# Orca0917/fine-grained-emotional-control-of-tts

Measured on AMD Instinct MI355X. Metric: train mel-frames/sec at B=32, 80-bin mel; 1/2/4/8 MI355X, higher is better.
Workload: dtype bf16; 1 GPU; FastSpeech2 train step (fwd+loss+bwd+allreduce+AdamW), B=32/GPU, T_phon_max=200, T_mel_max=977, D=384 F=1536 6+6 FFT layers, 80 mels; global_batch=32, seq_len=977, parallelism=dp1

## Files before the change

fine-grained-emotional-control-of-tts_amd/csrc/gemm.hip:

```cpp
#include <type_traits>

#include "fs2_cdna.h"
#include "fs2_launch.h"

#include <cstdlib>
#include <cstring>

namespace {

#ifdef FS2_EXPERIMENTS
#define XFLAGS(p) ((p).g4_flags)
#else
#define XFLAGS(p) 0
#endif

constexpr int BM = 128, BN = 128, NT = 256;
constexpr int TILE_BYTES = 128 * 128;

struct GemmP {
  int M, N, K, kvalid, mvalid, nvalid;
  const char* A; long lda; const char* B; long ldb;
  int conv_mode, conv_t, conv_kw, conv_c, conv_p;
  int conv_dil;
  char* C; long ldc; int c_fp32; int c_conv_kw;
// ... 2 lines not shown
  const float* row_scale;
  const char* residual; long ldr;
  const float* row_scale_post;
  int accumulate; int split_k; int k_per_split;
  long split_stride;
  int g4_flags;
  int batch_div;
  long sA1, sA2, sB1, sB2, sC1, sC2, sR1, sR2;
  int tiles_m, tiles_n;
  int vec_ok;
  int vec_align;
  int c_row_t, c_row_pad;
  int max_ctas;
  int a_bytes, b_bytes;
  int a_kw;
  const int32_t* k_eff;
};

__device__ __forceinline__ u32x4 add_bf16x8(u32x4 a, u32x4 b) {
  u32x4 r;
#pragma unroll
  for (int w = 0; w < 4; ++w) {
    float a0 = __builtin_bit_cast(float, a[w] << 16), a1 = __builtin_bit_cast(float, a[w] & 0xffff0000u);
    float b0 = __builtin_bit_cast(float, b[w] << 16), b1 = __builtin_bit_cast(float, b[w] & 0xffff0000u);
    bf16 r0 = (bf16)(a0 + b0), r1 = (bf16)(a1 + b1);
    r[w] = (unsigned)__builtin_bit_cast(unsigned short, r0) |
           ((unsigned)__builtin_bit_cast(unsigned short, r1) << 16);
  }
  return r;
}
__device__ __forceinline__ u32x4 add_f32x4(u32x4 a, u32x4 b) {
  const f32x4 fa = __builtin_bit_cast(f32x4, a), fb = __builtin_bit_cast(f32x4, b);
// ... 673 lines not shown
  const int z = p.split_k > 1 ? 0 : blockIdx.z;
  const long zb = z / p.batch_div, zh = z - zb * p.batch_div;
  const char* Ab = p.A + (zb * p.sA1 + zh * p.sA2) * 2;
  const char* Bb = p.B + (zb * p.sB1 + zh * p.sB2) * 2;
  const int K = p.K;
  const int kva = min(K, p.kvalid);
  const int amode = CM >= 0 ? CM : ((p.conv_mode == 1 || p.conv_mode == 4 || p.conv_mode == 5) ? p.conv_mode : 0);
  const int nk_all = (K + 63) / 64;
  int kt0 = 0, kt1 = nk_all;
  if (p.split_k > 1) {
    const int kps = (nk_all + p.split_k - 1) / p.split_k;
    kt0 = blockIdx.z * kps;
    kt1 = min(nk_all, kt0 + kps);
  }
  const bool bconv3 = B3 >= 0 ? B3 == 1 : p.conv_mode == 3;
  const bool tap_uniform = CM > 0 ? true : (CM == 0 ? false : amode && (p.conv_c % 64) == 0);
  const int rpu = amode == 4 ? p.conv_t + 2 * p.conv_p : p.conv_t;

  const i32x4 rsA = make_rsrc(Ab), rsB = make_rsrc(Bb);
  int avo[4];
  int abt[4], at[4], alc[4];
  bool aval[4];
#pragma unroll
  for (int i = 0; i < 4; ++i) {
    if constexpr (AK) {
      const int r = (wave * 4 + i) * 8 + (lane >> 3);
      alc[i] = (lane & 7) ^ (r & 7);
      const int row = m0 + r;
      aval[i] = row < p.M;
      const int rr = aval[i] ? row : 0;
// ... 126 lines not shown
        int ts = t + blc[i] - p.conv_p;
        ts = ts < 0 ? -ts : (ts >= p.conv_t ? 2 * (p.conv_t - 1) - ts : ts);
        const bool ok = bval[i] && k0 + bkr[i] < kva;
        const int vo = ok ? bvo[i] + (int)(((long)b * p.conv_t + ts) * p.ldb * 2) : BUF_OOB;
        blds16(rsB, vo, 0, lb + (wave * 2 + i) * 1024);
      }
    }
  };

  f32x4 acc[4][4];
#pragma unroll
  for (int i = 0; i < 4; ++i)
#pragma unroll
    for (int j = 0; j < 4; ++j) acc[i][j] = f32x4{0.f, 0.f, 0.f, 0.f};

  const int nk = kt1 - kt0;
  if (nk > 0) issue(kt0, 0);
  if (nk > 1) issue(kt0 + 1, 1);
  for (int it = 0; it < nk; ++it) {
    if (it + 1 < nk) asm volatile("s_waitcnt vmcnt(6)" ::: "memory");
    else asm volatile("s_waitcnt vmcnt(0)" ::: "memory");
    asm volatile("s_waitcnt lgkmcnt(0)" ::: "memory");
    __builtin_amdgcn_s_barrier();
    __builtin_amdgcn_sched_barrier(0);
    if (it + 2 < nk) issue(kt0 + it + 2, (it + 2) % 3);
    const char* la = smem + (it % 3) * BIG_STAGE;
    const char* lb = la + BIG_A;
    bf16x8 af[2][4], bfr[2][4];
#pragma unroll
    for (int s = 0; s < 2; ++s)
#pragma unroll
      for (int i = 0; i < 4; ++i) {
        af[s][i] = AK ? frag_bf16_kmajor(la, wm * 64 + i * 16, s, lane)
                      : frag_bf16_mnmajor_asm<512>(la, wm * 64 + i * 16, s, lane);
        bfr[s][i] = BKM ? frag_bf16_kmajor(lb, wn * 64 + i * 16, s, lane)
                        : frag_bf16_mnmajor_asm<256>(lb, wn * 64 + i * 16, s, lane);
      }
    if constexpr (!AK || !BKM) {
      asm volatile("s_waitcnt lgkmcnt(0)" ::: "memory");
#pragma unroll
// ... 67 lines not shown
  const int z = p.split_k > 1 ? 0 : blockIdx.z;
  const long zb = z / p.batch_div, zh = z - zb * p.batch_div;
  const char* Ab = p.A + (zb * p.sA1 + zh * p.sA2) * 2;
  const char* Bb = p.B + (zb * p.sB1 + zh * p.sB2) * 2;
  const int K = p.K;
  const int kva = min(K, p.kvalid);
  const int amode = CM >= 0 ? CM : ((p.conv_mode == 1 || p.conv_mode == 4 || p.conv_mode == 5) ? p.conv_mode : 0);
  const int nk_all = (K + 63) / 64;
  int kt0 = 0, kt1 = nk_all;
  if (p.split_k > 1) {
    const int kps = (nk_all + p.split_k - 1) / p.split_k;
    kt0 = blockIdx.z * kps;
    kt1 = min(nk_all, kt0 + kps);
  }
  const bool bconv3 = B3 >= 0 ? B3 == 1 : p.conv_mode == 3;
  const bool tap_uniform = CM > 0 ? true : (CM == 0 ? false : amode && (p.conv_c % 32) == 0);
  const int rpu = amode == 4 ? p.conv_t + 2 * p.conv_p : p.conv_t;

  const i32x4 rsA = make_rsrc(Ab), rsB = make_rsrc(Bb);
  int avo[2];
  int abt[2], at[2], ac[2];
  bool aval[2];
#pragma unroll
  for (int i = 0; i < 2; ++i) {
    const int piece = wave * 2 + i;
    if constexpr (AK) {
      const int r = piece * 16 + (lane >> 2);
      ac[i] = (lane & 3) ^ g4_fsw(r);
      const int row = m0 + r;
      aval[i] = row < p.M;
// ... 129 lines not shown
      const int dk = k0 - b_k;
      b_k = k0;
#pragma unroll
      for (int i = 0; i < 2; ++i) {
        int t = bt[i] + dk, b = bb[i];
        while (t >= p.conv_t) { t -= p.conv_t; ++b; }
        bt[i] = t; bb[i] = b;
        int ts = t + bc[i] - p.conv_p;
        ts = ts < 0 ? -ts : (ts >= p.conv_t ? 2 * (p.conv_t - 1) - ts : ts);
        const bool ok = bval[i] && k0 + bkr[i] < kva;
        const int vo = ok ? bvo[i] + (int)(((long)b * p.conv_t + ts) * p.ldb * 2) : BUF_OOB;
        blds16(rsB, vo, 0, dst + (wave * 2 + i) * 1024);
      }
    }
  };
  auto issue = [&](int it, int reg) {
    const int k0 = (kt0 + it) * 64 + (reg >> 1) * 32;
    char* dst = smem + (it & 1) * G4_SLOT + reg * G4_REG;
    if ((reg & 1) == 0) issueA(dst, k0);
    else issueB(dst, k0);
  };

  f32x4 acc[8][4];
#pragma unroll
  for (int i = 0; i < 8; ++i)
#pragma unroll
    for (int j = 0; j < 4; ++j) acc[i][j] = f32x4{0.f, 0.f, 0.f, 0.f};

  const int nk = kt1 - kt0;
  if (nk > 0) {
    issue(0, 1); issue(0, 0); issue(0, 3); issue(0, 2);
  }
  if (nk > 1) {
    issue(1, 1); issue(1, 0);
    asm volatile("s_waitcnt vmcnt(8)" ::: "memory");
  } else {
    asm volatile("s_waitcnt vmcnt(4)" ::: "memory");
  }
  __builtin_amdgcn_s_barrier();
  const bool stag = !(XFLAGS(p) & 1);
  const bool prio = !(XFLAGS(p) & 2);
  const bool nowait = XFLAGS(p) & 4;
  const bool noissue = XFLAGS(p) & 8;
  const int grp = stag ? wr : 1;
// ... 1518 lines not shown
  }
  constexpr int BIG_MIN_TILES = 60;
  const bool use_big = p.conv_mode != 2 &&
                       ((p.vec_ok && p.split_k <= 1 && tiles_big * batch >= BIG_MIN_TILES) ||
                        (slices && p.vec_ok && tiles_big * p.split_k >= 160) ||
                        (wgrad && tiles_big * split_big >= 160));
  if (!use_big) { pl.kernel = k128; return 0; }
  q.g4_flags = fs2_exp_int("FS2_BIG_FLAGS", 0);
  q.tiles_m = (p.M + BBM - 1) / BBM;
  if (wgrad) split_wgrad(split_big);
  pl.grid = dim3(q.tiles_m * q.tiles_n, 1, wgrad ? q.split_k : (slices ? p.split_k : gz));
  pl.kernel = K_BIG + tile_variant(ak, bk, conv_variant(q, 64), q.conv_mode);
  return 0;
}

int plan(const fs2_gemm_desc* d, GemmArgs& a, GemmPlan& pl) {
  const int rc = validate(d, a);
  return rc ? rc : plan_gemm(a, pl);
}

int launch(const GemmPlan& pl, hipStream_t s) {
  const GemmKernel& k = KERNELS[pl.kernel];
  hipLaunchKernelGGL(k.fn, pl.grid, dim3(k.block), 0, s, pl.p);
  FS2_CHECK_LAUNCH();
  return 0;
}

}

extern "C" int fs2_gemm(const fs2_gemm_desc* d, void* stream) {
  GemmArgs a;
  GemmPlan pl;
  if (const int rc = plan(d, a, pl)) return rc < 0 ? rc : 0;
  hipStream_t s = (hipStream_t)stream;
  const int oes = a.p.c_fp32 ? 4 : (a.dtype == FS2_BF16 ? 2 : 4);
  if (d->split_stride > 0)
    for (int z = a.p.split_k; z < d->split_k; ++z)
      if (hipMemset2DAsync(a.p.C + (long)z * d->split_stride * oes, a.p.ldc * oes, 0,
                           (size_t)a.p.nvalid * oes, a.p.mvalid, s) != hipSuccess)
        return FS2_EINVAL;
  return launch(pl, s);
}

extern "C" int fs2_gemm_plan(const fs2_gemm_desc* d, fs2_gemm_plan_info* out) {
  if (!out) return FS2_EINVAL;
  *out = fs2_gemm_plan_info{};
  GemmArgs a;
  GemmPlan pl;
  if (const int rc = plan(d, a, pl)) return rc < 0 ? rc : 0;
  std::strncpy(out->kernel, KERNELS[pl.kernel].name, sizeof(out->kernel) - 1);
  out->grid[0] = (int)pl.grid.x; out->grid[1] = (int)pl.grid.y; out->grid[2] = (int)pl.grid.z;
  out->block = KERNELS[pl.kernel].block;
  out->tiles_m = pl.p.tiles_m; out->tiles_n = pl.p.tiles_n;
  out->split_k = pl.p.split_k; out->k_per_split = pl.p.k_per_split;
  out->vec_ok = pl.p.vec_ok; out->accumulate = pl.p.accumulate;
  return 0;
}
```

fine-grained-emotional-control-of-tts_amd/csrc/norm.hip:

```cpp
#include <cstdlib>
#include <algorithm>
#include "fs2_launch.h"

namespace {

constexpr int MAXJ = 16;

template <bool DPP>
__device__ __forceinline__ float wsum(float v) {
  if constexpr (DPP) return wave_sum_dpp(v);
  else return wave_sum(v);
}

struct LnFwdP {
  const char* x; long ldx; const char* r; long ldr; float p_r; uint32_t salt_r;
  char* s_out; const float* gamma; const float* beta; float eps; int do_tanh;
  float p_o; uint32_t salt_o; const float* row_mask; const char* post_add; long ldp;
  char* y; long ldy; float* mean; float* rstd; int M, D; uint32_t seed;
  char* img; int img_t, img_p;
};

template <typename T>
__global__ void __launch_bounds__(256) ln_fwd_kernel(LnFwdP p) {
  const int lane = threadIdx.x & 63;
// ... 881 lines not shown
      const long v = (long)len[b] + halo;
      const int e = (int)(v < 0 ? 0 : (v > T ? T : v));
      w = fs2_km_width(b, e, T, P);
      if (end) end[b] = e;
    }
#pragma unroll
    for (int d = 1; d < 64; d <<= 1) {
      const int o = __shfl_up(w, d, 64);
      if (lane >= d) w += o;
    }
    if (offs && b < B) offs[b + 1] = carry + w;
    carry += __shfl(w, 63, 64);
  }
  if (offs)
    for (int i = B + 1 + lane; i < noffs; i += 64) offs[i] = 0x7fffffff;
}

__global__ void __launch_bounds__(256) pad_rows_kernel(const bf16* X, long ldx, int B, int T,
                                                       int C8, int P, int reflect, bf16* out,
                                                       long ldo, unsigned n8) {
  const unsigned idx = blockIdx.x * 256u + threadIdx.x;
  if (idx >= n8) return;
  const unsigned r = idx / (unsigned)C8;
  const int c = (int)(idx - r * (unsigned)C8) * 8;
  const unsigned L = (unsigned)(T + 2 * P);
  const unsigned b = r / L;
  const int i = (int)(r - b * L) - P;
  u32x4 v = {0u, 0u, 0u, 0u};
  if ((int)b < B) {
    const int t = reflect ? reflect_idx(i, T) : i;
// ... 233 lines not shown
                            ksplit, dtype, stream);
}

extern "C" int fs2_grad_tail_bounds(const int64_t* len, int B, int T, int halo, int P,
                                    int32_t* end, int32_t* offs, int noffs, void* stream) {
  if (B <= 0) return 0;
  if (!len || T <= 0 || halo < 0 || P < 0 || (!end && !offs)) return FS2_EINVAL;
  if (offs && (noffs < (B + 1 + 15) / 16 * 16 + 16 || (long)B * (T + 2L * P) >= 0x7fffffffL))
    return FS2_EINVAL;
  hipLaunchKernelGGL(grad_tail_bounds_kernel, dim3(1), dim3(64), 0, (hipStream_t)stream, len, B, T,
                     halo, P, end, offs, noffs);
  FS2_CHECK_LAUNCH();
  return 0;
}

extern "C" int fs2_pad_rows(const void* X, int64_t ldx, int B, int T, int C, int P, int reflect,
                            int tail, void* out, int64_t ldo, int dtype, void* stream) {
  if (B <= 0 || T <= 0 || C <= 0) return 0;
  if (dtype != FS2_BF16 || !X || !out || P < 0 || tail < 0 || (reflect && P >= T))
    return FS2_EINVAL;
  if ((C % 8) || (ldx % 8) || (ldo % 8) || ldo < C || ldx < C || !aligned16(X) || !aligned16(out))
    return FS2_EALIGN;
  const long rows = (long)B * (T + 2 * P) + tail;
  const long n8 = rows * (C / 8);
  if (n8 >= 0x7fffffffL || rows * ldo >= 0x7fffffffL) return FS2_EINVAL;
  hipLaunchKernelGGL(pad_rows_kernel, dim3((unsigned)((n8 + 255) / 256)), dim3(256), 0,
                     (hipStream_t)stream, (const bf16*)X, (long)ldx, B, T, C / 8, P, reflect,
                     (bf16*)out, (long)ldo, (unsigned)n8);
  FS2_CHECK_LAUNCH();
  return 0;
// ... 2 lines not shown
```

fine-grained-emotional-control-of-tts_amd/fastspeech2/_native.py:

```python

import ctypes
import os

import torch

_HERE = os.path.dirname(os.path.abspath(__file__))
LIB_PATH = os.environ.get("FS2_HIP_LIB", os.path.join(_HERE, "libfs2_hip.so"))
EXPERIMENTS = os.path.basename(LIB_PATH).startswith("libfs2_hip_exp")


def exp_flag(name, default=False):
    if not EXPERIMENTS:
        return default
    v = os.environ.get(name)
    return default if v is None else v not in ("", "0")


def exp_int(name, default):
    if not EXPERIMENTS:
        return default
    v = os.environ.get(name)
    return default if v is None else int(v)

F32 = 0
# ... 63 lines not shown
        ("O", ctypes.c_int), ("C", ctypes.c_int), ("KW", ctypes.c_int), ("w_okc", ctypes.c_int),
        ("ldf", ctypes.c_int), ("ldb", ctypes.c_int), ("tile0", ctypes.c_int),
        ("tiles_k", ctypes.c_int),
    ]


P = ctypes.c_void_p
I = ctypes.c_int
I64 = ctypes.c_int64
U32 = ctypes.c_uint32
Fl = ctypes.c_float

SIGNATURES = {
    "fs2_gemm": (I, [ctypes.POINTER(GemmDesc), P]),
    "fs2_gemm_plan": (I, [ctypes.POINTER(GemmDesc), ctypes.POINTER(GemmPlanInfo)]),
    "fs2_colsum": (I, [P, I64, I, I, I, P, I, P, P]),
    "fs2_conv_fold": (I, [P, I, I64, I, I, I, I, P, I64, P, I64, P, P, I, P]),
    "fs2_colsum_workspace_floats": (I64, [I, I]),
    "fs2_sum_slices": (I, [P, I, I64, I64, P, I, P]),
    "fs2_pad_transpose": (I, [P, I64, I, I, I, I, I, P, I64, I, P, P, I, P]),
    "fs2_pad_transpose_bounded": (I, [P, I64, I, I, I, I, I, P, I64, I, P, P, P, I, I, P]),
    "fs2_grad_tail_bounds": (I, [P, I, I, I, I, P, P, I, P]),
    "fs2_pad_rows": (I, [P, I64, I, I, I, I, I, I, P, I64, I, P]),
    "fs2_ln_fwd": (I, [P, I64, P, I64, Fl, U32, P, P, P, Fl, I, Fl, U32, P, P, I64, P, I64, P, P,
                       I, I, I, U32, P, I, I, P]),
    "fs2_ln_bwd": (I, [P, I64, P, I64, P, P, P, P, I, Fl, U32, P, I, P, I64, P, Fl, U32, P, P, P,
                       I, I, I, U32, P, P]),
    "fs2_ln_workspace_floats": (I64, [I, I]),
    "fs2_attn_supported": (I, [I, I, I]),
    "fs2_attn_fwd": (I, [P, I64, P, I, I, I, I, I, Fl, Fl, U32, U32, P, I64, P, I, P]),
# ... 142 lines not shown
```

fine-grained-emotional-control-of-tts_amd/fastspeech2/engine.py:

```python

import contextlib
import re

import torch

from . import _native as N
from . import ops
from .attention import attention_bwd, attention_fwd, use_flash
from .ops import round_up

BK = {N.F32: 32, N.BF16: 64}


class _Salt:
    def __init__(self):
        self.n = 0

    def __call__(self):
        self.n += 1
        return self.n


def dgrad_split(Mp, C, K, dt, n_cu=256, max_split=8):
    if dt != 1:
# ... 74 lines not shown
        self._wtable = None
        self.on_grads_ready = None
        self.timer = None
        self._km = {}
        self._offs = {}
        self._img = {}
        self._fimg = {}
        self.adam_split = None
        self._adam_late_done = False
        self.dp_late = None
        self.n_adam_late = 0
        self._adam_tabs = None
        self.skip_grad_tail = True
        self.check_grad_tail = False
        self.grad_tail_checked = []

    def _dec_halo(self):
        return sum((self._wspecs[f"decoder.layers.{i}.pos_ffn.{j}.conv.weight"][2] - 1) // 2
                   for i in range(self.cfg.dec_num_layers) for j in (0, 2))

    def _postnet_halo(self):
        return sum((kw - 1) // 2 for n, (_, _, kw) in self._wspecs.items()
                   if n.startswith("postnet."))

    def _tail_on(self):
        return self.skip_grad_tail or self.check_grad_tail

    def _km_offs(self, grad_end, P):
        ent = self._offs.get(id(grad_end))
        if ent is None or ent[0] is not grad_end or ent[1] != P:
            return None
        return ent[2]

    def _grad_end(self, mel_len, T, halo, P):
        end, offs = ops.grad_tail_bounds(mel_len.contiguous(), T, halo, P)
        self._offs[id(end)] = (end, P, offs)
        return end

    def _tail_bound(self, site, dy, B, T, grad_end, L=None):
        if grad_end is None:
            return None
        if self.check_grad_tail:
            L = L or T
            t = torch.arange(T, device=self.dev)[None, :] >= grad_end[:, None].long()
            tail = dy[:B * L].reshape(B, L, -1)[:, :T][t]
            nz = int((tail != 0).sum())
            assert nz == 0, f"{site}: {nz} non-zero gradient elements past grad_end"
            self.grad_tail_checked.append((site, int(tail.shape[0])))
        return grad_end if self.skip_grad_tail else None

    def _fwd_image(self, rows, tail, C):
        key = (rows, tail, C, self.adt)
# ... 342 lines not shown
        if isinstance(dY, tuple):
            img = dY[0]
            ops.gemm(Mp, C, KW * O, img, O, Wb, KW * O, Xpad, C, dt=self.dt, c_fp32=1,
                     split_k=split, split_stride=Mp * C if split > 1 else 0,
                     a_kw=KW if ti else 0)
        else:
            ops.gemm(Mp, C, KW * O, dY, lddy, Wb, KW * O, Xpad, C, dt=self.dt, conv=(4, T, KW, O),
                     c_fp32=1, split_k=split, split_stride=Mp * C if split > 1 else 0)
        assert set(epi) <= {"residual", "ldr", "row_scale", "row_scale_post"}, epi
        ops.conv_fold(Xpad, B, T, P, C, out, ldo, dt=self.dt, residual=epi.get("residual"),
                      ldr=epi.get("ldr", 0), row_scale=epi.get("row_scale"),
                      row_scale_post=epi.get("row_scale_post"), nsplit=split,
                      split_stride=Mp * C)

    def _wgrad(self, dY, lddy, X, ldx, M, T, wname, n_cols=None, gemm_tag=None, bias=None,
               dy_img=None, grad_end=None):
        grad_end = self._tail_bound(wname, dY, M // T, T, grad_end,
                                    T + self._wspecs[wname][2] - 1 if dy_img is not None else None)
        h = self._side_enter(dY, X, dy_img, grad_end)
        tag = self._dtag("wgrad", wname, T)
        if tag:
            self._tic(tag)
        ctas = self._side_ctas if h is not None else 0
        done = self._wgrad_impl(dY, lddy, X, ldx, M, T, wname, n_cols, gemm_tag, bias, dy_img,
                                ctas, grad_end)
        if tag:
            self._toc(tag)
        if bias is not None and not done:
            O = self._wspecs[wname][0]
            ops.colsum(dY, lddy, M, O, self.grads[bias], dt=self.dt, ws=self.ws(ops.colsum_ws(M, O)))
        self._side_exit(h)

    def _km_ok(self, O, C, KW, T, n_cols):
        return (self.dt == 1 and KW >= 5 and n_cols is None and
                C % 8 == 0 and O % 8 == 0 and (KW - 1) // 2 < T)

    def _km_image(self, key, C, ld):
        n = C * ld
        if torch.cuda.is_current_stream_capturing():
            return torch.zeros(n + 128, dtype=torch.bfloat16, device=self.dev)[64:64 + n]
# ... 37 lines not shown
                              ws=ws, **bk)
        ops.pad_transpose(X, ldx, B, T, C, P, 1, XT, Kp, Kp, dt=self.dt, **bk)
        stride = O * ncol
        ws = self.ws(S * stride)
        if gemm_tag:
            self._tic(gemm_tag)
        ops.gemm(O, ncol, Kp, dYT, Kp, XT, Kp, ws, ncol, dt=self.dt, conv=(6, T, KW, C),
                 c_fp32=1, split_k=S, split_stride=stride if S > 1 else 0, max_ctas=ctas,
                 k_eff=keff)
        if gemm_tag:
            self._toc(gemm_tag)
        ops.sum_slices(ws, S, stride, stride, self.grads[wname], accumulate=1)
        return True

    def _wgrad_impl(self, dY, lddy, X, ldx, M, T, wname, n_cols=None, gemm_tag=None, bias=None,
                    dy_img=None, ctas=0, grad_end=None):
        O, C, KW = self._wspecs[wname]
        if self._km_ok(O, C, KW, T, n_cols) and lddy % 8 == 0 and ldx % 8 == 0:
            return self._wgrad_km(dY, lddy, X, ldx, M, T, wname, gemm_tag, bias, dy_img, ctas,
                                  grad_end)
        if dy_img is not None:
            raise RuntimeError(f"{wname}: a padded dY image needs the K-major weight gradient")
        if n_cols is not None and n_cols != KW * C and KW == 1 and n_cols % 8 == 0 and self.dt == 1:
            K = round_up(M, self.epc)
            ns = eff_split(K, wgrad_slices(O, n_cols, n_cols, K, self.dt), BK[self.dt])
            ns = max(ns, 2)
            stride = O * n_cols
            ws = self.ws((ns + 1) * stride)
            ops.gemm(O, n_cols, K, dY, lddy, X, ldx, ws, n_cols, dt=self.dt, a_kmajor=0,
                     b_kmajor=0, c_fp32=1, kvalid=M, nvalid=n_cols, split_k=ns,
                     split_stride=stride, max_ctas=ctas)
            tot = ws[ns * stride:(ns + 1) * stride]
# ... 8 lines not shown
            split = max(1, min(-(-_WG_ATOMIC_UNITS // tiles), K // (BK[self.dt] * 4)))
        conv = (3, T, KW, C) if KW > 1 else None
        ldc = C * KW
        ns = wgrad_slices(O, Ncols, ldc, K, self.dt, _WG_SLICE_CU)
        if ns == 1 and self.dt == 1 and Ncols == ldc and O * ldc > 600_000:
            tiles = -(-O // 256) * -(-Ncols // 256)
            ns = max(1, min(-(-_SLICE_TARGET // tiles), (K // 64) // 8))
        ns = eff_split(K, ns, BK[self.dt])
        if ns > 1:
            stride = O * ldc
            ws = self.ws(ns * stride)
            if gemm_tag:
                self._tic(gemm_tag)
            ops.gemm(O, Ncols, K, dY, lddy, X, ldx, ws, ldc, dt=self.dt, a_kmajor=0, b_kmajor=0,
                     conv=conv, c_fp32=1, kvalid=M, nvalid=ldc, split_k=ns, split_stride=stride,
                     max_ctas=ctas)
            if gemm_tag:
                self._toc(gemm_tag)
            ops.sum_slices(ws, ns, stride, stride, self.grads[wname], accumulate=1)
            return
        ops.gemm(O, Ncols, K, dY, lddy, X, ldx, self.grads[wname], ldc, dt=self.dt, a_kmajor=0,
                 b_kmajor=0, conv=conv, c_fp32=1, kvalid=M, nvalid=KW * C, accumulate=1,
                 split_k=split, max_ctas=ctas)

    def _bias_grad(self, dY, lddy, M, n, gname):
        h = self._side_enter(dY)
        ops.colsum(dY, lddy, M, n, self.grads[gname], dt=self.dt, ws=self.ws(ops.colsum_ws(M, n)))
        self._side_exit(h)

    def _fft_fwd(self, X, B, T, key_pad, prefix, H, p_drop, seed, salt):
        D = self.cfg.enc_d_model
        M = B * T
        P = self.params
        ctx = {"X": X}
        QKV = self.empty(M, 3 * D)
        self._fwd(X, D, M, T, prefix + "self_att.att.in_proj_weight", QKV, 3 * D,
                  bias=P[prefix + "self_att.att.in_proj_bias"])
        Att = self.empty(M, D)
# ... 51 lines not shown
                   dbeta=G[prefix + "norm2.norm.bias"], dcol=G[prefix + "pos_ffn.2.conv.bias"])
        w2 = prefix + "pos_ffn.2.conv.weight"
        w1 = prefix + "pos_ffn.0.conv.weight"
        pad = self._pad_dgrad(w1)
        if pad and not self._pad_dgrad_fits(w1, B, T):
            raise ValueError(f"{w1}: batch of {B} x {T} tokens exceeds the 32-bit offsets of the "
                             "padded conv data gradient; split the batch")
        if pad:
            P1 = (self._wspecs[w1][2] - 1) // 2
            img, dHc = self._dy_image(prefix, B, T, P1, F)
            crow = {"c_row": (T, 2 * P1)}
        else:
            img, crow = None, {}
            dHc = self.empty(M, F)
        dX1 = self.empty(M, D)
        self._wgrad(dY, D, ctx["Hc"], F, M, T, w2)
        self._dgrad(dY, D, M, T, w2, dHc, F, gate=ctx["Hc"], ldg=F, **crow)
        self._wgrad(dHc, F, ctx["X1"], D, M, T, w1,
                    gemm_tag="ffn_conv1_wgrad." + prefix.split(".")[0],
                    bias=prefix + "pos_ffn.0.conv.bias", dy_img=img, grad_end=grad_end)
        self._dgrad((img,) if pad else dHc, F, M, T, w1, dX1, D, residual=ds2, ldr=D)
        del dY, dHc, ds2, img
        lnws = self.ws(ops.ln_ws(M, D))
        ds1, dAo = self.empty(M, D), self.empty(M, D)
        ops.ln_bwd(dX1, D, ctx["s1"], D, ctx["mean1"], ctx["rstd1"], P[prefix + "norm1.norm.weight"],
                   P[prefix + "norm1.norm.bias"], ds1, D, M, D, dt=self.dt, ws=lnws, seed=seed,
                   dr=dAo, p_r=p_drop, salt_r=ctx["s_r1"], dgamma=G[prefix + "norm1.norm.weight"],
                   dbeta=G[prefix + "norm1.norm.bias"],
                   dcol=G[prefix + "self_att.att.out_proj.bias"])
        del dX1
        wo = prefix + "self_att.att.out_proj.weight"
        dAtt = self.empty(M, D)
        self._wgrad(dAo, D, ctx["Att"], D, M, T, wo)
        self._dgrad(dAo, D, M, T, wo, dAtt, D)
        del dAo
        dQKV = self.empty(M, 3 * D)
        qb = self._tail_bound(prefix + "attn_bwd", dAtt, B, T, grad_end) if "lse" in ctx else None
        attention_bwd(ctx["QKV"], ctx["key_pad"], ctx["Att"], dAtt, ctx, B, H, T, D, dQKV,
                      dt=self.dt, dev=self.dev, mask_mode=1, p_drop=p_drop, seed=seed,
                      salt=ctx["s_att"], empty=self.empty, ws=self.ws, q_bound=qb,
                      timed=self._timed("attn_bwd", T))
        wi = prefix + "self_att.att.in_proj_weight"
        dX = self.empty(M, D)
        self._wgrad(dQKV, 3 * D, ctx["X"], D, M, T, wi)
        self._bias_grad(dQKV, 3 * D, M, 3 * D, prefix + "self_att.att.in_proj_bias")
        self._dgrad(dQKV, 3 * D, M, T, wi, dX, D, residual=ds1, ldr=D)
        return dX

    def _pred_fwd(self, Zin, keep, B, T, name, rate, p_drop, seed, salt, a1=None, lda1=None,
                  salts=None):
        D = self.cfg.enc_d_model
        M = B * T
        P = self.params
        c = {"Zin": Zin}
        if a1 is None:
            a1, lda1 = self.empty(M, D), D
            self._fwd(Zin, D, M, T, name + ".conv1.conv.weight", a1, D,
                      bias=P[name + ".conv1.conv.bias"], relu=1)
        v1 = self.empty(M, D)
# ... 352 lines not shown
        dmel = self._postnet_bwd(d_post, d_mel_total, keep_m, ctx["pn_ctx"], B, Tm, ctx["p_post"],
                                 seed, ctx["mel_len"])
        notify("postnet")
        dXo = self.empty(Mm, D)
        self._dgrad(dmel, NM, Mm, Tm, "linear.w.weight", dXo, D)
        self._wgrad(dmel, NM, ctx["Xo"], D, Mm, Tm, "linear.w.weight")
        self._bias_grad(dmel, NM, Mm, NM, "linear.w.bias")
        dX = self.empty(Mm, D)
        ops.ln_bwd(dXo, D, ctx["Xdec_last"], D, ctx["md"], ctx["rd"], P["decoder.norm.norm.weight"],
                   P["decoder.norm.norm.bias"], dX, D, Mm, D, dt=self.dt, ws=self.ws(ops.ln_ws(Mm, D)),
                   dgamma=G["decoder.norm.norm.weight"], dbeta=G["decoder.norm.norm.bias"])
        notify("linear")
        dec_end = None
        if self._tail_on():
            P1 = (self._wspecs["decoder.layers.0.pos_ffn.0.conv.weight"][2] - 1) // 2
            dec_end = self._grad_end(ctx["mel_len"], Tm, self._dec_halo(), P1)
        for i in reversed(range(c.dec_num_layers)):
            dX = self._fft_bwd(dX, ctx["dec_ctx"][i], B, Tm, f"decoder.layers.{i}.", H_d,
                               ctx["p_dec"], seed, grad_end=dec_end)
            notify(f"decoder.layers.{i}")
        dZ3 = self.empty(Mp, D)
        ops.lr_scatter(dX, ctx["cum"], keep_m, B, Tp, Tm, D, dZ3, dt=self.dt)
        def wg_side(fn, *tensors):
            h = self._side_enter(*tensors)
            fn()
            self._side_exit(h)
        kwe = c.energy_pred_kernel_size
        wg_side(lambda: ops.embed1d_bwd(dZ3, ctx["a_e"], B, Tp, D, kwe, G["energyEmbed.conv.weight"],
                                        G["energyEmbed.conv.bias"], dt=self.dt,
                                        ws=self.ws(128 * (kwe + 1) * D)), dZ3, ctx["a_e"])
        if dZe is not None:
# ... 46 lines not shown
```

fine-grained-emotional-control-of-tts_amd/fastspeech2/ops.py:

```python

import collections
import ctypes
import os
import sys

import torch

from . import _native as N

EPC = {N.F32: 4, N.BF16: 8}


def _p(x):
    if x is None:
        return None
    if isinstance(x, int):
        return x
    return x.data_ptr()


def _s():
    return N.stream_ptr()


def _chk(rc, name):
    if rc != 0:
        raise RuntimeError(f"{name} returned {rc}")


def round_up(x, m):
    return (x + m - 1) // m * m


_TRACE = collections.Counter() if os.environ.get("FS2_GEMM_TRACE") else None

GemmPlan = collections.namedtuple(
    "GemmPlan", "kernel grid block tiles_m tiles_n split_k k_per_split vec_ok accumulate")


def _plan(d):
    i = N.GemmPlanInfo()
    _chk(N.lib().fs2_gemm_plan(ctypes.byref(d), ctypes.byref(i)), "fs2_gemm_plan")
    return GemmPlan(i.kernel.decode(), tuple(i.grid), i.block, i.tiles_m, i.tiles_n, i.split_k,
                    i.k_per_split, i.vec_ok, i.accumulate)


def _trace(d):
    f = sys._getframe(2)
    while f is not None and os.path.basename(f.f_code.co_filename) == "ops.py":
        f = f.f_back
    site = f"{f.f_code.co_name}:{f.f_lineno}" if f is not None else "?"
    flags = "".join(k for k, v in (("a", not d.a_kmajor), ("b", not d.b_kmajor), ("f", d.c_fp32),
                                   ("B", d.bias), ("r", d.relu), ("g", d.gate), ("R", d.residual),
                                   ("s", d.row_scale), ("S", d.row_scale_post),
                                   ("+", d.accumulate), ("c", d.c_row_t)) if v)
    pl = _plan(d)
    _TRACE[(d.M, d.N, d.K, d.conv_mode, d.split_k, d.batch, flags, pl.kernel, pl.grid, site)] += 1
# ... 3 lines not shown
    for k, n in sorted(_TRACE.items(), key=lambda x: -x[0][0] * x[0][1] * x[0][2] * x[1]):
        M, N_, K, cm, sk, b, fl, kern, grid, site = k
        print(f"gemm {n:4d}x M {M:6d} N {N_:5d} K {K:6d} conv {cm} split {sk} batch {b:4d} "
              f"[{fl}] {kern} grid {grid[0]}x{grid[2]} {site}", file=sys.stderr)


if _TRACE is not None:
    import atexit
    atexit.register(_trace_dump)


def gemm(M, N_, K, A, lda, B, ldb, C, ldc, *, dt, a_kmajor=1, b_kmajor=1, conv=None, c_fp32=0,
         c_conv_kw=0, bias=None, relu=0, gate=None, ldg=0, row_scale=None, residual=None, ldr=0,
         row_scale_post=None, accumulate=0, split_k=1, split_stride=0, kvalid=0, mvalid=0,
         nvalid=0, batch=1, batch_div=1, strides=None, conv_dil=1, c_row=None, max_ctas=0,
         a_kw=0, k_eff=None, plan=False):
    d = N.GemmDesc()
    d.k_eff = _p(k_eff)
    d.conv_dil = conv_dil
    d.a_kw = a_kw
    d.max_ctas = max_ctas
    if c_row is not None:
        d.c_row_t, d.c_row_pad = c_row
    d.M, d.N, d.K, d.kvalid, d.mvalid, d.nvalid, d.dtype = M, N_, K, kvalid, mvalid, nvalid, dt
    d.A, d.lda, d.a_kmajor = _p(A), lda, a_kmajor
    d.B, d.ldb, d.b_kmajor = _p(B), ldb, b_kmajor
    if conv is not None:
        d.conv_mode, d.conv_t, d.conv_kw, d.conv_c = conv
    d.C, d.ldc, d.c_fp32, d.c_conv_kw = _p(C), ldc, c_fp32, c_conv_kw
    d.bias, d.relu = _p(bias), relu
    d.gate, d.ldg = _p(gate), ldg
    d.row_scale = _p(row_scale)
    d.residual, d.ldr = _p(residual), ldr
    d.row_scale_post = _p(row_scale_post)
    d.accumulate, d.split_k, d.split_stride = accumulate, split_k, split_stride
    d.batch, d.batch_div = batch, batch_div
    if strides is not None:
        (d.sA1, d.sA2, d.sB1, d.sB2, d.sC1, d.sC2, d.sR1, d.sR2) = strides
    if plan:
        return _plan(d)
    if _TRACE is not None:
        _trace(d)
    _chk(N.lib().fs2_gemm(ctypes.byref(d), _s()), "fs2_gemm")


def gemm_plan(*args, **kw):
    return gemm(*args, plan=True, **kw)


def conv_fold(Xpad, B, T, P, C, out, ldo, *, dt, residual=None, ldr=0, row_scale=None,
              row_scale_post=None, nsplit=1, split_stride=0):
    _chk(N.lib().fs2_conv_fold(_p(Xpad), nsplit, split_stride, B, T, P, C, _p(out), ldo,
                               _p(residual), ldr,
                               _p(row_scale), _p(row_scale_post), dt, _s()), "fs2_conv_fold")


def grad_tail_bounds(mel_len, T, halo, P):
    B = mel_len.numel()
    assert mel_len.dtype == torch.int64 and mel_len.is_contiguous()
    end = torch.empty(B, dtype=torch.int32, device=mel_len.device)
    offs = torch.empty(round_up(B + 1, 16) + 16, dtype=torch.int32, device=mel_len.device)
    _chk(N.lib().fs2_grad_tail_bounds(_p(mel_len), B, T, halo, P, _p(end), _p(offs), offs.numel(),
                                      _s()), "fs2_grad_tail_bounds")
    return end, offs


_TRI = {}


def km_offsets(grad_end, T, P):
    B = grad_end.numel()
    key = (B, grad_end.device)
    tri = _TRI.get(key)
    if tri is None:
        tri = torch.ones(B, B, dtype=torch.int32, device=grad_end.device).tril()
        if not torch.cuda.is_current_stream_capturing():
            _TRI[key] = tri
    offs = torch.full((round_up(B + 1, 16) + 16,), 2 ** 31 - 1, dtype=torch.int32,
                      device=grad_end.device)
# ... 363 lines not shown
```

include/fs2_hip.h:

```cpp
#ifndef FS2_HIP_H
#define FS2_HIP_H

#include <stdint.h>

#ifdef __cplusplus
extern "C" {
#endif

#define FS2_F32 0
#define FS2_BF16 1

#define FS2_EINVAL (-1)
#define FS2_EALIGN (-2)

typedef struct fs2_gemm_desc {
  int M, N, K;
  int kvalid;
  int mvalid, nvalid;
  int dtype;
  const void* A; int64_t lda; int a_kmajor;
  const void* B; int64_t ldb; int b_kmajor;
  int conv_mode, conv_t, conv_kw, conv_c;
  void* C; int64_t ldc; int c_fp32;
  int c_conv_kw;
// ... 16 lines not shown
} fs2_gemm_desc;

int fs2_gemm(const fs2_gemm_desc* d, void* stream);

typedef struct fs2_gemm_plan_info {
  char kernel[64];
  int grid[3];
  int block;
  int tiles_m, tiles_n;
  int split_k, k_per_split;
  int vec_ok, accumulate;
} fs2_gemm_plan_info;

int fs2_gemm_plan(const fs2_gemm_desc* d, fs2_gemm_plan_info* out);

int fs2_conv_fold(const float* Xpad, int nsplit, int64_t split_stride, int B, int T, int P,
                  int C, void* out, int64_t ldo, const void* residual, int64_t ldr,
                  const float* row_scale, const float* row_scale_post, int dtype, void* stream);

int fs2_pad_transpose(const void* X, int64_t ldx, int B, int T, int C, int P, int reflect,
                      void* out, int64_t ldo, int ncols, float* colsum, float* workspace,
                      int dtype, void* stream);
int fs2_pad_transpose_bounded(const void* X, int64_t ldx, int B, int T, int C, int P, int reflect,
                              void* out, int64_t ldo, int ncols, float* colsum, float* workspace,
                              const int32_t* offs, int ksplit, int dtype, void* stream);

int fs2_grad_tail_bounds(const int64_t* len, int B, int T, int halo, int P, int32_t* end,
                         int32_t* offs, int noffs, void* stream);

int fs2_sum_slices(const float* ws, int nslices, int64_t stride, int64_t n, float* out,
                   int accumulate, void* stream);

int fs2_pad_rows(const void* X, int64_t ldx, int B, int T, int C, int P, int reflect, int tail,
                 void* out, int64_t ldo, int dtype, void* stream);

int fs2_colsum(const void* X, int64_t ldx, int M, int N, int dtype, float* out, int accumulate,
               float* workspace, void* stream);
int64_t fs2_colsum_workspace_floats(int M, int N);

int fs2_ln_fwd(const void* x, int64_t ldx, const void* r, int64_t ldr, float p_r, uint32_t salt_r,
               void* s_out, const float* gamma, const float* beta, float eps, int do_tanh,
               float p_o, uint32_t salt_o, const float* row_mask, const void* post_add,
               int64_t ldp, void* y, int64_t ldy, float* mean, float* rstd, int M, int D,
// ... 187 lines not shown
```

Before: 1.537 million mel-frames/s.

## Skip all-padding K tiles in decoder 1x1 weight-gradient GEMMs via live-tile table

A small kernel builds, from the per-sequence gradient end bounds, a table of 64-row K tiles that contain any non-padded mel frames, plus prefix counts. The MN-major bf16 GEMM kernels (big and 256 variants) load that table and iterate only over the live K tiles, using readlane to fetch each tile index. Decoder out_proj, in_proj and FFN conv2 weight-gradient calls pass this table, so they avoid MMA and loads on padded time steps whose gradient is zero. The cost is one extra tiny launch, a per-CTA global load at kernel start, and the requirement that split ranges span at most 64 tiles.

```diff
diff --git a/fine-grained-emotional-control-of-tts_amd/csrc/gemm.hip b/fine-grained-emotional-control-of-tts_amd/csrc/gemm.hip
--- a/fine-grained-emotional-control-of-tts_amd/csrc/gemm.hip
+++ b/fine-grained-emotional-control-of-tts_amd/csrc/gemm.hip
@@ -40,8 +40,21 @@
   int max_ctas;
   int a_bytes, b_bytes;
   int a_kw;
-  const int32_t* k_eff;
+  union {
+    const int32_t* k_eff;
+    const int32_t* k_live;
+  };
 };
+
+__device__ __forceinline__ int k_live_stage(const int32_t* tab, int nk_all, int kt0, int kt1,
+                                            int lane, int& ktab) {
+  const int base = tab[kt0];
+  const int n = tab[kt1] - base;
+  const int32_t* src = tab + nk_all + 1 + min(base + lane, nk_all - 1);
+  asm volatile("global_load_dword %0, %1, off\n\ts_waitcnt vmcnt(0)"
+               : "=&v"(ktab) : "v"(src) : "memory");
+  return n;
+}
 
 __device__ __forceinline__ u32x4 add_bf16x8(u32x4 a, u32x4 b) {
   u32x4 r;
@@ -745,6 +758,7 @@
     kt1 = min(nk_all, kt0 + kps);
   }
   const bool bconv3 = B3 >= 0 ? B3 == 1 : p.conv_mode == 3;
+  constexpr bool KL = !AK && !BKM && CM == 0 && B3 == 0;
   const bool tap_uniform = CM > 0 ? true : (CM == 0 ? false : amode && (p.conv_c % 64) == 0);
   const int rpu = amode == 4 ? p.conv_t + 2 * p.conv_p : p.conv_t;
 
@@ -901,16 +915,30 @@
 #pragma unroll
     for (int j = 0; j < 4; ++j) acc[i][j] = f32x4{0.f, 0.f, 0.f, 0.f};
 
-  const int nk = kt1 - kt0;
-  if (nk > 0) issue(kt0, 0);
-  if (nk > 1) issue(kt0 + 1, 1);
+  int nk = kt1 - kt0;
+  int ktab = 0;
+  bool listed = false;
+  if constexpr (KL) {
+    if (p.k_live) {
+      listed = true;
+      nk = k_live_stage(p.k_live, nk_all, kt0, kt1, lane, ktab);
+    }
+  }
+  auto tile = [&](int it, int ahead) {
+    if constexpr (KL) {
+      if (listed) return __builtin_amdgcn_readlane(ktab, it + ahead);
+    }
+    return kt0 + it + ahead;
+  };
+  if (nk > 0) issue(tile(0, 0), 0);
+  if (nk > 1) issue(tile(0, 1), 1);
   for (int it = 0; it < nk; ++it) {
     if (it + 1 < nk) asm volatile("s_waitcnt vmcnt(6)" ::: "memory");
     else asm volatile("s_waitcnt vmcnt(0)" ::: "memory");
     asm volatile("s_waitcnt lgkmcnt(0)" ::: "memory");
     __builtin_amdgcn_s_barrier();
     __builtin_amdgcn_sched_barrier(0);
-    if (it + 2 < nk) issue(kt0 + it + 2, (it + 2) % 3);
+    if (it + 2 < nk) issue(tile(it, 2), (it + 2) % 3);
     const char* la = smem + (it % 3) * BIG_STAGE;
     const char* lb = la + BIG_A;
     bf16x8 af[2][4], bfr[2][4];
@@ -1008,6 +1036,7 @@
     kt1 = min(nk_all, kt0 + kps);
   }
   const bool bconv3 = B3 >= 0 ? B3 == 1 : p.conv_mode == 3;
+  constexpr bool KL = !AK && !BKM && CM == 0 && B3 == 0;
   const bool tap_uniform = CM > 0 ? true : (CM == 0 ? false : amode && (p.conv_c % 32) == 0);
   const int rpu = amode == 4 ? p.conv_t + 2 * p.conv_p : p.conv_t;
 
@@ -1167,8 +1196,23 @@
       }
     }
   };
+  int nk = kt1 - kt0;
+  int ktab = 0;
+  bool listed = false;
+  if constexpr (KL) {
+    if (p.k_live) {
+      listed = true;
+      nk = k_live_stage(p.k_live, nk_all, kt0, kt1, lane, ktab);
+    }
+  }
+  auto tile = [&](int it) {
+    if constexpr (KL) {
+      if (listed) return __builtin_amdgcn_readlane(ktab, it);
+    }
+    return kt0 + it;
+  };
   auto issue = [&](int it, int reg) {
-    const int k0 = (kt0 + it) * 64 + (reg >> 1) * 32;
+    const int k0 = tile(it) * 64 + (reg >> 1) * 32;
     char* dst = smem + (it & 1) * G4_SLOT + reg * G4_REG;
     if ((reg & 1) == 0) issueA(dst, k0);
     else issueB(dst, k0);
@@ -1180,7 +1224,6 @@
 #pragma unroll
     for (int j = 0; j < 4; ++j) acc[i][j] = f32x4{0.f, 0.f, 0.f, 0.f};
 
-  const int nk = kt1 - kt0;
   if (nk > 0) {
     issue(0, 1); issue(0, 0); issue(0, 3); issue(0, 2);
   }
@@ -2729,9 +2772,21 @@
   return 0;
 }
 
-int plan(const fs2_gemm_desc* d, GemmArgs& a, GemmPlan& pl) {
-  const int rc = validate(d, a);
-  return rc ? rc : plan_gemm(a, pl);
+int attach_k_live(const fs2_gemm_desc* d, const GemmArgs& a, GemmPlan& pl, const int32_t* k_live) {
+  if (!k_live) return 0;
+  if (a.dtype != FS2_BF16 || a.ak || a.bk || d->conv_mode || a.batch > 1) return FS2_EINVAL;
+  const int row = tile_variant(0, 0, 0, 0);
+  const int nk_all = (pl.p.K + 63) / 64;
+  const int kps = pl.p.split_k > 1 ? (nk_all + pl.p.split_k - 1) / pl.p.split_k : nk_all;
+  if ((pl.kernel == K_BIG + row || pl.kernel == K_256 + row - 1) && kps <= 64)
+    pl.p.k_live = k_live;
+  return 0;
+}
+
+int plan(const fs2_gemm_desc* d, GemmArgs& a, GemmPlan& pl, const int32_t* k_live = nullptr) {
+  int rc = validate(d, a);
+  if (!rc) rc = plan_gemm(a, pl);
+  return rc ? rc : attach_k_live(d, a, pl, k_live);
 }
 
 int launch(const GemmPlan& pl, hipStream_t s) {
@@ -2741,12 +2796,10 @@
   return 0;
 }
 
-}
-
-extern "C" int fs2_gemm(const fs2_gemm_desc* d, void* stream) {
+int gemm_run(const fs2_gemm_desc* d, const int32_t* k_live, void* stream) {
   GemmArgs a;
   GemmPlan pl;
-  if (const int rc = plan(d, a, pl)) return rc < 0 ? rc : 0;
+  if (const int rc = plan(d, a, pl, k_live)) return rc < 0 ? rc : 0;
   hipStream_t s = (hipStream_t)stream;
   const int oes = a.p.c_fp32 ? 4 : (a.dtype == FS2_BF16 ? 2 : 4);
   if (d->split_stride > 0)
@@ -2757,12 +2810,12 @@
   return launch(pl, s);
 }
 
-extern "C" int fs2_gemm_plan(const fs2_gemm_desc* d, fs2_gemm_plan_info* out) {
+int gemm_plan_info(const fs2_gemm_desc* d, const int32_t* k_live, fs2_gemm_plan_info* out) {
   if (!out) return FS2_EINVAL;
   *out = fs2_gemm_plan_info{};
   GemmArgs a;
   GemmPlan pl;
-  if (const int rc = plan(d, a, pl)) return rc < 0 ? rc : 0;
+  if (const int rc = plan(d, a, pl, k_live)) return rc < 0 ? rc : 0;
   std::strncpy(out->kernel, KERNELS[pl.kernel].name, sizeof(out->kernel) - 1);
   out->grid[0] = (int)pl.grid.x; out->grid[1] = (int)pl.grid.y; out->grid[2] = (int)pl.grid.z;
   out->block = KERNELS[pl.kernel].block;
@@ -2771,3 +2824,20 @@
   out->vec_ok = pl.p.vec_ok; out->accumulate = pl.p.accumulate;
   return 0;
 }
+
+}
+
+extern "C" int fs2_gemm(const fs2_gemm_desc* d, void* stream) { return gemm_run(d, nullptr, stream); }
+
+extern "C" int fs2_gemm_plan(const fs2_gemm_desc* d, fs2_gemm_plan_info* out) {
+  return gemm_plan_info(d, nullptr, out);
+}
+
+extern "C" int fs2_gemm_k_live(const fs2_gemm_desc* d, const int32_t* k_live, void* stream) {
+  return gemm_run(d, k_live, stream);
+}
+
+extern "C" int fs2_gemm_k_live_plan(const fs2_gemm_desc* d, const int32_t* k_live,
+                                    fs2_gemm_plan_info* out) {
+  return gemm_plan_info(d, k_live, out);
+}
diff --git a/fine-grained-emotional-control-of-tts_amd/csrc/norm.hip b/fine-grained-emotional-control-of-tts_amd/csrc/norm.hip
--- a/fine-grained-emotional-control-of-tts_amd/csrc/norm.hip
+++ b/fine-grained-emotional-control-of-tts_amd/csrc/norm.hip
@@ -919,6 +919,28 @@
   }
   if (offs)
     for (int i = B + 1 + lane; i < noffs; i += 64) offs[i] = 0x7fffffff;
+}
+
+__global__ void __launch_bounds__(64) live_k_tiles_kernel(const int32_t* end, int T, int M, int nk,
+                                                          int32_t* tab) {
+  const int lane = threadIdx.x;
+  int32_t* live = tab + nk + 1;
+  int carry = 0;
+  for (int k0 = 0; k0 < nk; k0 += 64) {
+    const int k = k0 + lane;
+    bool on = false;
+    if (k < nk) {
+      const int r0 = k * 64, r1 = min(r0 + 63, M - 1);
+      for (int b = r0 / T; b <= r1 / T && !on; ++b) on = max(r0 - b * T, 0) < end[b];
+    }
+    const unsigned long long m = __ballot(on);
+    const int below = carry + __popcll(m & ((1ull << lane) - 1ull));
+    if (k < nk) tab[k] = below;
+    if (on) live[below] = k;
+    carry += __popcll(m);
+  }
+  if (lane == 0) tab[nk] = carry;
+  for (int i = carry + lane; i < nk; i += 64) live[i] = nk;
 }
 
 __global__ void __launch_bounds__(256) pad_rows_kernel(const bf16* X, long ldx, int B, int T,
@@ -1182,6 +1204,17 @@
   return 0;
 }
 
+extern "C" int fs2_live_k_tiles(const int32_t* end, int B, int T, int M, int32_t* table,
+                                void* stream) {
+  if (B <= 0) return 0;
+  if (!end || !table || T <= 0 || (long)B * T != M || M > 0x7fffff00) return FS2_EINVAL;
+  const int nk = (int)(((long)M + 63) / 64);
+  hipLaunchKernelGGL(live_k_tiles_kernel, dim3(1), dim3(64), 0, (hipStream_t)stream, end, T, M,
+                     nk, table);
+  FS2_CHECK_LAUNCH();
+  return 0;
+}
+
 extern "C" int fs2_pad_rows(const void* X, int64_t ldx, int B, int T, int C, int P, int reflect,
                             int tail, void* out, int64_t ldo, int dtype, void* stream) {
   if (B <= 0 || T <= 0 || C <= 0) return 0;
diff --git a/fine-grained-emotional-control-of-tts_amd/fastspeech2/_native.py b/fine-grained-emotional-control-of-tts_amd/fastspeech2/_native.py
--- a/fine-grained-emotional-control-of-tts_amd/fastspeech2/_native.py
+++ b/fine-grained-emotional-control-of-tts_amd/fastspeech2/_native.py
@@ -101,6 +101,9 @@
 SIGNATURES = {
     "fs2_gemm": (I, [ctypes.POINTER(GemmDesc), P]),
     "fs2_gemm_plan": (I, [ctypes.POINTER(GemmDesc), ctypes.POINTER(GemmPlanInfo)]),
+    "fs2_gemm_k_live": (I, [ctypes.POINTER(GemmDesc), P, P]),
+    "fs2_gemm_k_live_plan": (I, [ctypes.POINTER(GemmDesc), P, ctypes.POINTER(GemmPlanInfo)]),
+    "fs2_live_k_tiles": (I, [P, I, I, I, P, P]),
     "fs2_colsum": (I, [P, I64, I, I, I, P, I, P, P]),
     "fs2_conv_fold": (I, [P, I, I64, I, I, I, I, P, I64, P, I64, P, P, I, P]),
     "fs2_colsum_workspace_floats": (I64, [I, I]),
diff --git a/fine-grained-emotional-control-of-tts_amd/fastspeech2/engine.py b/fine-grained-emotional-control-of-tts_amd/fastspeech2/engine.py
--- a/fine-grained-emotional-control-of-tts_amd/fastspeech2/engine.py
+++ b/fine-grained-emotional-control-of-tts_amd/fastspeech2/engine.py
@@ -112,6 +112,7 @@
         self.skip_grad_tail = True
         self.check_grad_tail = False
         self.grad_tail_checked = []
+        self.grad_tail_checked_k = []
 
     def _dec_halo(self):
         return sum((self._wspecs[f"decoder.layers.{i}.pos_ffn.{j}.conv.weight"][2] - 1) // 2
@@ -130,10 +131,24 @@
             return None
         return ent[2]
 
-    def _grad_end(self, mel_len, T, halo, P):
+    def _grad_end(self, mel_len, T, halo, P, k_tiles=False):
         end, offs = ops.grad_tail_bounds(mel_len.contiguous(), T, halo, P)
-        self._offs[id(end)] = (end, P, offs)
+        self._offs[id(end)] = (end, P, offs, ops.live_k_tiles(end, T) if k_tiles else None)
         return end
+
+    def _k_live(self, site, dy, B, T, k_end):
+        if k_end is None:
+            return None
+        if self.check_grad_tail:
+            t = torch.arange(T, device=self.dev)[None, :] >= k_end[:, None].long()
+            tail = dy[:B * T].reshape(B, T, -1)[t]
+            nz = int((tail != 0).sum())
+            assert nz == 0, f"{site}: {nz} non-zero gradient elements past grad_end"
+            self.grad_tail_checked_k.append((site, int(tail.shape[0])))
+        ent = self._offs.get(id(k_end))
+        if not self.skip_grad_tail or ent is None or ent[0] is not k_end:
+            return None
+        return ent[3]
 
     def _tail_bound(self, site, dy, B, T, grad_end, L=None):
         if grad_end is None:
@@ -506,16 +521,17 @@
                       split_stride=Mp * C)
 
     def _wgrad(self, dY, lddy, X, ldx, M, T, wname, n_cols=None, gemm_tag=None, bias=None,
-               dy_img=None, grad_end=None):
+               dy_img=None, grad_end=None, k_end=None):
         grad_end = self._tail_bound(wname, dY, M // T, T, grad_end,
                                     T + self._wspecs[wname][2] - 1 if dy_img is not None else None)
-        h = self._side_enter(dY, X, dy_img, grad_end)
+        k_live = self._k_live(wname, dY, M // T, T, k_end)
+        h = self._side_enter(dY, X, dy_img, grad_end, k_live)
         tag = self._dtag("wgrad", wname, T)
         if tag:
             self._tic(tag)
         ctas = self._side_ctas if h is not None else 0
         done = self._wgrad_impl(dY, lddy, X, ldx, M, T, wname, n_cols, gemm_tag, bias, dy_img,
-                                ctas, grad_end)
+                                ctas, grad_end, k_live)
         if tag:
             self._toc(tag)
         if bias is not None and not done:
@@ -583,8 +599,10 @@
         return True
 
     def _wgrad_impl(self, dY, lddy, X, ldx, M, T, wname, n_cols=None, gemm_tag=None, bias=None,
-                    dy_img=None, ctas=0, grad_end=None):
+                    dy_img=None, ctas=0, grad_end=None, k_live=None):
         O, C, KW = self._wspecs[wname]
+        if not (self.dt == 1 and KW == 1 and n_cols is None):
+            k_live = None
         if self._km_ok(O, C, KW, T, n_cols) and lddy % 8 == 0 and ldx % 8 == 0:
             return self._wgrad_km(dY, lddy, X, ldx, M, T, wname, gemm_tag, bias, dy_img, ctas,
                                   grad_end)
@@ -623,14 +641,14 @@
                 self._tic(gemm_tag)
             ops.gemm(O, Ncols, K, dY, lddy, X, ldx, ws, ldc, dt=self.dt, a_kmajor=0, b_kmajor=0,
                      conv=conv, c_fp32=1, kvalid=M, nvalid=ldc, split_k=ns, split_stride=stride,
-                     max_ctas=ctas)
+                     max_ctas=ctas, k_live=k_live)
             if gemm_tag:
                 self._toc(gemm_tag)
             ops.sum_slices(ws, ns, stride, stride, self.grads[wname], accumulate=1)
             return
         ops.gemm(O, Ncols, K, dY, lddy, X, ldx, self.grads[wname], ldc, dt=self.dt, a_kmajor=0,
                  b_kmajor=0, conv=conv, c_fp32=1, kvalid=M, nvalid=KW * C, accumulate=1,
-                 split_k=split, max_ctas=ctas)
+                 split_k=split, max_ctas=ctas, k_live=k_live)
 
     def _bias_grad(self, dY, lddy, M, n, gname):
         h = self._side_enter(dY)
@@ -712,7 +730,7 @@
             img, crow = None, {}
             dHc = self.empty(M, F)
         dX1 = self.empty(M, D)
-        self._wgrad(dY, D, ctx["Hc"], F, M, T, w2)
+        self._wgrad(dY, D, ctx["Hc"], F, M, T, w2, k_end=grad_end)
         self._dgrad(dY, D, M, T, w2, dHc, F, gate=ctx["Hc"], ldg=F, **crow)
         self._wgrad(dHc, F, ctx["X1"], D, M, T, w1,
                     gemm_tag="ffn_conv1_wgrad." + prefix.split(".")[0],
@@ -729,7 +747,7 @@
         del dX1
         wo = prefix + "self_att.att.out_proj.weight"
         dAtt = self.empty(M, D)
-        self._wgrad(dAo, D, ctx["Att"], D, M, T, wo)
+        self._wgrad(dAo, D, ctx["Att"], D, M, T, wo, k_end=grad_end)
         self._dgrad(dAo, D, M, T, wo, dAtt, D)
         del dAo
         dQKV = self.empty(M, 3 * D)
@@ -740,7 +758,7 @@
                       timed=self._timed("attn_bwd", T))
         wi = prefix + "self_att.att.in_proj_weight"
         dX = self.empty(M, D)
-        self._wgrad(dQKV, 3 * D, ctx["X"], D, M, T, wi)
+        self._wgrad(dQKV, 3 * D, ctx["X"], D, M, T, wi, k_end=grad_end)
         self._bias_grad(dQKV, 3 * D, M, 3 * D, prefix + "self_att.att.in_proj_bias")
         self._dgrad(dQKV, 3 * D, M, T, wi, dX, D, residual=ds1, ldr=D)
         return dX
@@ -1123,7 +1141,7 @@
         dec_end = None
         if self._tail_on():
             P1 = (self._wspecs["decoder.layers.0.pos_ffn.0.conv.weight"][2] - 1) // 2
-            dec_end = self._grad_end(ctx["mel_len"], Tm, self._dec_halo(), P1)
+            dec_end = self._grad_end(ctx["mel_len"], Tm, self._dec_halo(), P1, k_tiles=True)
         for i in reversed(range(c.dec_num_layers)):
             dX = self._fft_bwd(dX, ctx["dec_ctx"][i], B, Tm, f"decoder.layers.{i}.", H_d,
                                ctx["p_dec"], seed, grad_end=dec_end)
diff --git a/fine-grained-emotional-control-of-tts_amd/fastspeech2/ops.py b/fine-grained-emotional-control-of-tts_amd/fastspeech2/ops.py
--- a/fine-grained-emotional-control-of-tts_amd/fastspeech2/ops.py
+++ b/fine-grained-emotional-control-of-tts_amd/fastspeech2/ops.py
@@ -38,9 +38,13 @@
     "GemmPlan", "kernel grid block tiles_m tiles_n split_k k_per_split vec_ok accumulate")
 
 
-def _plan(d):
+def _plan(d, k_live=None):
     i = N.GemmPlanInfo()
-    _chk(N.lib().fs2_gemm_plan(ctypes.byref(d), ctypes.byref(i)), "fs2_gemm_plan")
+    if k_live is None:
+        _chk(N.lib().fs2_gemm_plan(ctypes.byref(d), ctypes.byref(i)), "fs2_gemm_plan")
+    else:
+        _chk(N.lib().fs2_gemm_k_live_plan(ctypes.byref(d), _p(k_live), ctypes.byref(i)),
+             "fs2_gemm_k_live_plan")
     return GemmPlan(i.kernel.decode(), tuple(i.grid), i.block, i.tiles_m, i.tiles_n, i.split_k,
                     i.k_per_split, i.vec_ok, i.accumulate)
 
@@ -74,7 +78,7 @@
          c_conv_kw=0, bias=None, relu=0, gate=None, ldg=0, row_scale=None, residual=None, ldr=0,
          row_scale_post=None, accumulate=0, split_k=1, split_stride=0, kvalid=0, mvalid=0,
          nvalid=0, batch=1, batch_div=1, strides=None, conv_dil=1, c_row=None, max_ctas=0,
-         a_kw=0, k_eff=None, plan=False):
+         a_kw=0, k_eff=None, k_live=None, plan=False):
     d = N.GemmDesc()
     d.k_eff = _p(k_eff)
     d.conv_dil = conv_dil
@@ -98,9 +102,12 @@
     if strides is not None:
         (d.sA1, d.sA2, d.sB1, d.sB2, d.sC1, d.sC2, d.sR1, d.sR2) = strides
     if plan:
-        return _plan(d)
+        return _plan(d, k_live)
     if _TRACE is not None:
         _trace(d)
+    if k_live is not None:
+        _chk(N.lib().fs2_gemm_k_live(ctypes.byref(d), _p(k_live), _s()), "fs2_gemm_k_live")
+        return
     _chk(N.lib().fs2_gemm(ctypes.byref(d), _s()), "fs2_gemm")
 
 
@@ -123,6 +130,15 @@
     _chk(N.lib().fs2_grad_tail_bounds(_p(mel_len), B, T, halo, P, _p(end), _p(offs), offs.numel(),
                                       _s()), "fs2_grad_tail_bounds")
     return end, offs
+
+
+def live_k_tiles(end, T):
+    B = end.numel()
+    assert end.dtype == torch.int32 and end.is_contiguous()
+    nk = (B * T + 63) // 64
+    tab = torch.empty(2 * nk + 1, dtype=torch.int32, device=end.device)
+    _chk(N.lib().fs2_live_k_tiles(_p(end), B, T, B * T, _p(tab), _s()), "fs2_live_k_tiles")
+    return tab
 
 
 _TRI = {}
diff --git a/include/fs2_hip.h b/include/fs2_hip.h
--- a/include/fs2_hip.h
+++ b/include/fs2_hip.h
@@ -54,6 +54,9 @@
 
 int fs2_gemm_plan(const fs2_gemm_desc* d, fs2_gemm_plan_info* out);
 
+int fs2_gemm_k_live(const fs2_gemm_desc* d, const int32_t* k_live, void* stream);
+int fs2_gemm_k_live_plan(const fs2_gemm_desc* d, const int32_t* k_live, fs2_gemm_plan_info* out);
+
 int fs2_conv_fold(const float* Xpad, int nsplit, int64_t split_stride, int B, int T, int P,
                   int C, void* out, int64_t ldo, const void* residual, int64_t ldr,
                   const float* row_scale, const float* row_scale_post, int dtype, void* stream);
@@ -67,6 +70,7 @@
 
 int fs2_grad_tail_bounds(const int64_t* len, int B, int T, int halo, int P, int32_t* end,
                          int32_t* offs, int noffs, void* stream);
+int fs2_live_k_tiles(const int32_t* end, int B, int T, int M, int32_t* table, void* stream);
 
 int fs2_sum_slices(const float* ws, int nslices, int64_t stride, int64_t n, float* out,
                    int accumulate, void* stream);
```

Result: no change. 1.545 million mel-frames/s, median of 6 (+0.5%).
